# dazzmo/ik

Hardware: AMD Instinct MI355X
Metric: IK solves/sec (50-iter DLS) at batch=65536 (higher is better)
Workload: dtype f64; 1 GPU; Cassie single-leg chain (cassie_fixed.urdf, 7 support joints of nq=16), one SE(3) LeftFootFront task, 50 fixed DLS iterations, damping 1e-2, step 1.0, reachable targets FK(q*); batch_per_gpu=65536, global_batch=65536, kernel=dls_chain<NJ=7,full,hot>, parallelism=single GPU

## Files before the change

### ik_amd/csrc/capi.cpp

```cpp
#include <hip/hip_runtime.h>

#include <time.h>

#include <algorithm>
#include <cmath>
#include <cstdio>
#include <cstdlib>
#include <cstring>
#include <exception>
#include <memory>
#include <mutex>
#include <new>
#include <stdexcept>
#include <string>
#include <type_traits>
#include <vector>

#include "ikgpu.h"
#include "kernels.hpp"
#include "model.hpp"
#include "problem.hpp"

namespace {

// ... 64 lines not shown

struct ikgpu_problem {
    mutable Staging stage;
    mutable HostPipe pipe;
    ikgpu::ProblemHost host;
    ikgpu::ProblemHost gen;
    ikgpu::DeviceTables dev;
    int device = 0;
    int nframes = 0;
    bool dls_on_static_gen = false;
    mutable std::once_flag visitor_static_once;
    mutable uint64_t visitor_static_key = 0;
    mutable bool visitor_static = false;
    mutable std::once_flag pik_static_once[2];
    mutable uint64_t pik_static_key[2] = {0, 0};
    mutable bool pik_static[2] = {false, false};
    std::vector<uint8_t> draw;
    std::string dls_name;
    std::string pik_name;
    std::string pik_tree_name;
    std::string pik_static_name;
    explicit ikgpu_problem(int device_) : device(device_) {}
    ~ikgpu_problem() {
        DeviceGuard g(device);
        void *const tables[] = {dev.lower, dev.upper, dev.q_in_chain, dev.draw, dev.chain_desc, dev.g_ints, dev.g_dbls};
        for (void *t : tables) (void)hipFree(t);
        dev.queues.release();
        pipe.release();
        stage.release();
    }
};
static_assert(!std::is_copy_constructible<Staging>::value && !std::is_copy_constructible<HostPipe>::value &&
                  !std::is_copy_constructible<ikgpu_problem>::value && !std::is_copy_assignable<ikgpu_problem>::value,
              "owners of device memory must not be copyable");

namespace {

thread_local std::string g_last_error;

bool shape_built(const ikgpu::ProblemHost &ph) {
    if (ph.kind == ikgpu::KernelKind::Generic) return true;
    return ph.kind == ikgpu::KernelKind::Chain ? ikgpu::chain_shape_built(ph.chain.nj, ph.tasks[0].type)
                                               : ikgpu::tree_shape_built(ph.chain.nj, ph.chainB.nj > 0 ? 2 : 1);
}

ikgpu::ProblemHost analyse(const ikgpu::Model &m, const ikgpu_task *tasks, int32_t ntasks, const ikgpu_task *cons, int32_t ncons,
                           bool compile_rtc) {
    const char *force = std::getenv("IKGPU_DLS_KERNEL");
    ikgpu::ProblemHost ph = ikgpu::analyse_problem(m, tasks, ntasks, force && std::strcmp(force, "generic") == 0, cons, ncons);
    if (!shape_built(ph)) ph = ikgpu::analyse_problem(m, tasks, ntasks, true, cons, ncons);
    if (ph.kind == ikgpu::KernelKind::Chain) {
        ph.chain_build = ikgpu::select_chain_build(ph, compile_rtc);
        ph.kernel_name = ikgpu::chain_kernel_name(ph);
    }
    if (ph.kind == ikgpu::KernelKind::Generic && ikgpu::rtc_generic_static_available(ph, compile_rtc, &ph.generic_key)) {
        ph.generic_build = 2;
        ph.kernel_name = ph.kernel_name.substr(0, ph.kernel_name.size() - 1) + ",static>";
    }
    return ph;
}

int fail(int code, const std::string &msg) {
    g_last_error = msg;
    return code;
}

bool tree_prefers_static(const ikgpu::ProblemHost &ph) {
    if (ph.kind != ikgpu::KernelKind::Tree) return false;
    long rows = 12;
    if (const char *env = std::getenv("IKGPU_TREE_STATIC_ROWS")) rows = std::strtol(env, nullptr, 10);
    if (ph.cons_on && !std::getenv("IKGPU_TREE_STATIC_CONSTRAINED")) return false;
    return ikgpu::rtc_static_solve_rows(ph) <= rows;
}

std::string static_name(const ikgpu::ProblemHost &gen) {
    const std::string &n = gen.kernel_name;
    return n.size() > 8 && n.compare(n.size() - 8, 8, ",static>") == 0 ? n : n.substr(0, n.size() - 1) + ",static>";
}

struct KernelPlan {
    ikgpu::ProblemHost host, gen;
    bool dls_on_static_gen = false;
    std::string name;
};
KernelPlan plan_kernels(const ikgpu::Model &m, const ikgpu_task *tasks, int32_t ntasks, const ikgpu_task *cons, int32_t ncons, bool compile) {
    KernelPlan k;
    k.host = analyse(m, tasks, ntasks, cons, ncons, compile);
    k.gen = k.host.kind == ikgpu::KernelKind::Generic ? k.host : ikgpu::analyse_problem(m, tasks, ntasks, true, cons, ncons);
    k.name = k.host.kernel_name;
    if (tree_prefers_static(k.host) && ikgpu::rtc_generic_static_available(k.gen, compile, &k.gen.generic_key)) {
        k.gen.generic_build = 2;
        k.dls_on_static_gen = true;
        k.name = static_name(k.gen);
    }
    return k;
}

}

int ikgpu_set_last_error(int code, const std::string &msg) { return fail(code, msg); }

namespace {

int hip_fail(hipError_t e, const char *what) {
    return fail(IKGPU_ERR_DEVICE, std::string(what) + ": " + hipGetErrorString(e));
}
// ... 1363 lines not shown
```

### ik_amd/csrc/device/chain_hot.hpp

```cpp
#pragma once
#if !defined(__HIPCC_RTC__)
#include <cstdint>
#endif

#include "chain_kernel_body.hpp"

namespace ikdev {

constexpr int kStructBits = 21;
constexpr int kStructPerWord = 3;
enum : unsigned { kEntGeneral = 0, kEntZero = 1, kEntOne = 2, kEntMinusOne = 3 };

template <uint64_t C0, uint64_t C1, uint64_t C2, unsigned PM = 0>
struct ChainStruct {
    static constexpr unsigned kPrismatic = PM;
    static constexpr bool prismatic(int j) { return j >= 0 && ((PM >> j) & 1u) != 0; }
    static constexpr uint64_t word(int w) { return w == 0 ? C0 : (w == 1 ? C1 : C2); }
    static constexpr unsigned code(int i) { return static_cast<unsigned>((word(i / kStructPerWord) >> (kStructBits * (i % kStructPerWord))) & 0x1fffffu); }
    static constexpr unsigned ent(int i, int e) { return (code(i) >> (2 * e)) & 3u; }
    static constexpr bool tnz(int i, int k) { return ((code(i) >> (18 + k)) & 1u) != 0; }
    static constexpr int ngen_before(int i, int e) { return e == 0 ? 0 : ngen_before(i, e - 1) + (ent(i, e - 1) == kEntGeneral ? 1 : 0); }
    static constexpr int count(int i) { return ngen_before(i, 9) + (tnz(i, 0) ? 1 : 0) + (tnz(i, 1) ? 1 : 0) + (tnz(i, 2) ? 1 : 0); }
    static constexpr int offset(int i) { return i == 0 ? 0 : offset(i - 1) + count(i - 1); }
    static constexpr int rot_at(int i, int e) { return offset(i) + ngen_before(i, e); }
// ... 37 lines not shown
};

struct HotLutNoStage {};
#if IKD_HIP_LANG
typedef double SinCosPair __attribute__((ext_vector_type(2)));
static __device__ const double kSinCosLutDevice[2 * IKD_SINCOS_LUT_SIZE] __attribute__((aligned(16), unused)) = {IKD_SINCOS_LUT_VALUES};
struct HotTableLds : HotTable {
    SinCosPair *lut;
};
constexpr int kHotLutPerLane = IKD_SINCOS_LUT_SIZE / 64;
struct HotLutStage { SinCosPair v[kHotLutPerLane]; };
__device__ __forceinline__ HotLutStage hot_lut_issue(const HotTableLds &) {
    HotLutStage st;
    const SinCosPair *src = reinterpret_cast<const SinCosPair *>(kSinCosLutDevice);
    const int lane = static_cast<int>(threadIdx.x) & 63;
#pragma unroll
    for (int i = 0; i < kHotLutPerLane; ++i) st.v[i] = src[lane + 64 * i];
    return st;
}
__device__ __forceinline__ void hot_lut_commit(const HotTableLds &t, const HotLutStage &st) {
    const int lane = static_cast<int>(threadIdx.x) & 63;
#pragma unroll
    for (int i = 0; i < kHotLutPerLane; ++i) t.lut[lane + 64 * i] = st.v[i];
    __builtin_amdgcn_fence(__ATOMIC_RELEASE, "workgroup");
    __builtin_amdgcn_wave_barrier();
    __builtin_amdgcn_fence(__ATOMIC_ACQUIRE, "workgroup");
}
__device__ __forceinline__ void hot_lut_fetch(const HotTableLds &t, int idx, double &S, double &C) {
    const SinCosPair e = t.lut[idx];
    S = e.x;
    C = e.y;
}
#define IKD_HOT_LUT_DECLARE(tv)                                       \
    __shared__ SinCosPair ikd_hot_lut[IKD_SINCOS_LUT_SIZE];           \
    HotTableLds tv;                                                   \
    tv.lut = ikd_hot_lut
#endif
IKD_FN HotLutNoStage hot_lut_issue(const HotTable &) { return HotLutNoStage{}; }
IKD_FN void hot_lut_commit(const HotTable &, const HotLutNoStage &) {}
#if IKD_ON_DEVICE && !defined(IKD_HOT_LUT_FROM_HBM)
void hot_lut_fetch(const HotTable &, int idx, double &S, double &C) = delete;
#else
IKD_FN void hot_lut_fetch(const HotTable &, int idx, double &S, double &C) {
#if IKD_ON_DEVICE
    S = kSinCosLutDevice[2 * idx];
    C = kSinCosLutDevice[2 * idx + 1];
#else
    S = kSinCosLutHost[2 * idx];
    C = kSinCosLutHost[2 * idx + 1];
#endif
}
#endif

template <int NJ, unsigned PM = 0, class Tab>
IKD_FN void hot_sincos(const Tab &t, const double (&phi)[NJ], double (&sn)[NJ], double (&cs)[NJ]) {
    double res[NJ], tS[NJ], tC[NJ], sl[NJ], cm1[NJ];
    int idx[NJ];
#pragma unroll
    for (int j = 0; j < NJ; ++j)
        if (!((PM >> j) & 1u)) dsincos_lut_reduce(phi[j], res[j], idx[j]);
#pragma unroll
    for (int j = NJ - 1; j >= 0; --j)
        if (!((PM >> j) & 1u)) hot_lut_fetch(t, idx[j], tS[j], tC[j]);
    IKD_SCHED_FENCE();
#pragma unroll
    for (int j = 0; j < NJ; ++j)
        if (!((PM >> j) & 1u)) dsincos_lut_poly(res[j], sl[j], cm1[j]);
#pragma unroll
    for (int j = NJ - 1; j >= 0; --j)
        if (!((PM >> j) & 1u)) dsincos_lut_combine(tS[j], tC[j], sl[j], cm1[j], sn[j], cs[j]);
}

template <class S, int I, class Tab>
IKD_FN double hot_rot(const Tab &t, int e) {
    return S::ent(I, e) == kEntGeneral ? t.v[S::rot_at(I, e)] : S::literal(I, e);
}

template <class S, int I, class Tab>
IKD_FN void hot_compose_left(double (&R)[9], double (&p)[3], const Tab &t) {
    double Ro[9], po[3];
#pragma unroll
    for (int k = 0; k < 9; ++k) Ro[k] = R[k];
#pragma unroll
    for (int k = 0; k < 3; ++k) po[k] = p[k];
#pragma unroll
    for (int r = 0; r < 3; ++r) {
        const double c0 = hot_rot<S, I>(t, 3 * r), c1 = hot_rot<S, I>(t, 3 * r + 1), c2 = hot_rot<S, I>(t, 3 * r + 2);
#pragma unroll
        for (int k = 0; k < 3; ++k) R[3 * r + k] = dfma(c0, Ro[k], dfma(c1, Ro[3 + k], c2 * Ro[6 + k]));
        const double last = S::tnz(I, r) ? dfma(c2, po[2], t.v[S::trans_at(I, r)]) : c2 * po[2];
        p[r] = dfma(c0, po[0], dfma(c1, po[1], last));
    }
}

template <class S, class Tab>
IKD_FN void hot_fold_base(const Tab &t, const double (&oMt)[12], double (&oM0)[12]) {
    double c[9], dp[3];
#pragma unroll
    for (int k = 0; k < 9; ++k) c[k] = hot_rot<S, 0>(t, k);
#pragma unroll
    for (int k = 0; k < 3; ++k) dp[k] = S::tnz(0, k) ? oMt[9 + k] - t.v[S::trans_at(0, k)] : oMt[9 + k];
#pragma unroll
    for (int i = 0; i < 3; ++i) {
#pragma unroll
        for (int j = 0; j < 3; ++j) oM0[3 * i + j] = dfma(c[i], oMt[j], dfma(c[3 + i], oMt[3 + j], c[6 + i] * oMt[6 + j]));
        oM0[9 + i] = dfma(c[i], dp[0], dfma(c[3 + i], dp[1], c[6 + i] * dp[2]));
    }
}

template <int NJ, class S, bool BASE_FOLDED = false, class Tab>
IKD_FN void hot_evaluate(const Tab &t, const double (&q)[NJ], const double (&oMt)[12], double (&e)[6], double (&col)[NJ][6]) {
    constexpr typename ChainRuns<S, NJ>::Table kRuns = ChainRuns<S, NJ>::value;
    double phi[NJ], sn[NJ], cs[NJ];
#pragma unroll
    for (int j = NJ - 1; j >= 0; --j) phi[j] = (kRuns.folded[j] && !kRuns.tip[j]) ? phi[j + 1 < NJ ? j + 1 : j] + q[j] : q[j];
    hot_sincos<NJ, S::kPrismatic>(t, phi, sn, cs);

    double ang[NJ][3], lin[NJ][3];
    double rows[NJ][6], pt[NJ][2];
    double R[9], p[3];
// ... 150 lines not shown
IKD_FN void hot_step(const Tab &t, const LoopParams &prm, const double (&col)[NJ][6], const double (&y)[6], double (&q)[NJ], bool take) {
    constexpr int kLim = S::offset(NJ + 1);
    constexpr typename ChainRuns<S, NJ>::Table kRuns = ChainRuns<S, NJ>::value;
    double ang[NJ];
#pragma unroll
    for (int j = 0; j < NJ; ++j)
        if (kRuns.leader[j] == j && !kRuns.prismatic[j]) ang[j] = dfma(col[j][3], y[3], dfma(col[j][4], y[4], col[j][5] * y[5]));
#pragma unroll
    for (int j = 0; j < NJ; ++j) {
        double s = kRuns.prismatic[j] ? 0.0 : ang[kRuns.leader[j]];
#pragma unroll
        for (int a = 0; a < 3; ++a) s = dfma(col[j][a], y[a], s);
        const double qn = dfma(prm.step_length, s, q[j]);
        const double qc = dmin(t.v[kLim + NJ + j], dmax(qn, t.v[kLim + j]));
        q[j] = take ? qc : q[j];
    }
}

template <int NJ, class S, bool NEVERSTOP, class Tab, class AnyFn>
IKD_FN void hot_dls(const Tab &t, const LoopParams &prm, double (&q)[NJ], const double (&oMt)[12], int &iters_out,
                    bool &success_out, AnyFn any_active, bool active = true) {
    constexpr int M = 6;
    bool success = false;
    int iters = prm.max_iterations;
    double oM0[12];
    hot_fold_base<S>(t, oMt, oM0);
#pragma unroll 1
    for (int it = 0; it < prm.max_iterations; ++it) {
        double e[M], col[NJ][M];
        hot_evaluate<NJ, S, true>(t, q, oM0, e, col);

        double G[M * M];
        hot_gram<NJ, S>(col, prm.lam2, G);
        double y[M];
        ldlt_solve<M>(G, e, y);

        if (!NEVERSTOP) {
            double e0sq = 0.0;
            if (prm.priority == 0) {
#pragma unroll
                for (int a = 0; a < M; ++a) e0sq = dfma(e[a], e[a], e0sq);
            }
            const bool stop_now = active && (prm.stop_sq_tol >= 0.0) && (e0sq < prm.stop_sq_tol);
            if (stop_now) { success = true; iters = it; }
            active = active && !stop_now;
        }
        hot_step<NJ, S>(t, prm, col, y, q, NEVERSTOP || active);
        if (!NEVERSTOP && !any_active(active)) break;
    }
    iters_out = (NEVERSTOP || success) ? iters : iterations_taken(any_active, prm.max_iterations);
    success_out = success;
}

template <int NJ>
IKD_FN void hot_pass_through_from(const ChainKernelArgs<NJ> &a, const double *q_src, double *q_out, int64_t b, bool stepped) {
    const ChainStrides st = chain_strides(a);
    constexpr int kGroup = 16;
    for (int i0 = 0; i0 < a.nq; i0 += kGroup) {
        double v[kGroup], lo[kGroup], hi[kGroup];
        bool out[kGroup];
#pragma unroll
        for (int k = 0; k < kGroup; ++k) {
            const int i = i0 + k < a.nq ? i0 + k : a.nq - 1;
            out[k] = i0 + k < a.nq && !a.q_in_chain[i];
            lo[k] = a.lower[i];
            hi[k] = a.upper[i];
        }
#pragma unroll
        for (int k = 0; k < kGroup; ++k) {
            const int i = i0 + k < a.nq ? i0 + k : a.nq - 1;
            v[k] = q_src[at(st.elem, st.q_prob, i, b)];
        }
#pragma unroll
        for (int k = 0; k < kGroup; ++k) {
            const double c = dmin(hi[k], dmax(v[k], lo[k]));
            if (out[k]) q_out[at(st.elem, st.q_prob, i0 + k, b)] = stepped ? c : v[k];
        }
    }
}
template <int NJ>
IKD_FN void hot_pass_through_to(const ChainKernelArgs<NJ> &a, double *q_out, int64_t b, bool stepped) { hot_pass_through_from(a, a.q0, q_out, b, stepped); }
template <int NJ>
IKD_FN void hot_pass_through(const ChainKernelArgs<NJ> &a, int64_t b, bool stepped) { hot_pass_through_to(a, a.q_out, b, stepped); }

#if IKD_HIP_LANG
template <int NJ, class S, class Tab>
__device__ __forceinline__ void hot_refill_body(const ChainKernelArgs<NJ> &a, const Tab &t, unsigned long long *queue, int chunk) {
    struct Stage {
        const Tab &t;
        decltype(hot_lut_issue(t)) st;
        __device__ __forceinline__ void issue() { st = hot_lut_issue(t); }
        __device__ __forceinline__ void commit() { hot_lut_commit(t, st); }
    };
    chain_refill_loop<NJ>(a, queue, chunk, [&](double (&q)[NJ], const double (&oMt)[12], bool have) {
        constexpr int M = 6;
        double e[M], col[NJ][M];
        hot_evaluate<NJ, S, true>(t, q, oMt, e, col);
        double G[M * M];
        hot_gram<NJ, S>(col, a.prm.lam2, G);
        double y[M];
        ldlt_solve<M>(G, e, y);
        double e0sq = 0.0;
        if (a.prm.priority == 0) {
#pragma unroll
            for (int k = 0; k < M; ++k) e0sq = dfma(e[k], e[k], e0sq);
        }
        const bool stop_now = have && (a.prm.stop_sq_tol >= 0.0) && (e0sq < a.prm.stop_sq_tol);
        hot_step<NJ, S>(t, a.prm, col, y, q, !stop_now);
        return stop_now;
    }, [&](double (&oMt)[12]) {
        double w[12];
#pragma unroll
        for (int k = 0; k < 12; ++k) w[k] = oMt[k];
        hot_fold_base<S>(t, w, oMt);
    }, Stage{t, {}});
}
#endif

template <int NJ, class S, bool NEVERSTOP, class Tab, class AnyFn>
IKD_FN void hot_chain_body(const ChainKernelArgs<NJ> &a, const Tab &t, int64_t gid, AnyFn any_active, long long wave_start = 0) {
    const ChainStrides st = chain_strides(a);
#if defined(IKGPU_HOT_STAMP) && IKD_ON_DEVICE
    const long long rs = wave_start;
#endif
    const bool valid = gid < a.B;
    const int64_t b = valid ? gid : a.B - 1;
    const auto lut_stage = hot_lut_issue(t);
    double q[NJ];
#pragma unroll
    for (int j = 0; j < NJ; ++j) q[j] = a.q0[at(st.elem, st.q_prob, a.qidx[j], b)];
    double oMt[12];
    load_target(a, b, oMt);
    hot_lut_commit(t, lut_stage);
    if (NEVERSTOP && valid) hot_pass_through(a, b, a.prm.max_iterations > 0);
    int iters;
    bool success;
#if defined(IKGPU_HOT_STAMP) && IKD_ON_DEVICE
    const long long c0 = __builtin_readcyclecounter(), r0 = wall_clock64();
#endif
    hot_dls<NJ, S, NEVERSTOP>(t, a.prm, q, oMt, iters, success, any_active);
#if defined(IKGPU_HOT_STAMP) && IKD_ON_DEVICE
    const long long c1 = __builtin_readcyclecounter(), r1 = wall_clock64();
    const int stamp_loop_cycles = static_cast<int>(c1 - c0), stamp_loop_ticks = static_cast<int>(r1 - r0);
    const int stamp_pre_ticks = static_cast<int>(r0 - rs);
    const int stamp_true_iters = iters;
#endif
    if (!NEVERSTOP && a.append_count)
        append_unfinished(a.append_list, a.append_count, valid && !success && iters < a.prm.max_iterations, b);
    if (!valid) return;
#pragma unroll
    for (int j = 0; j < NJ; ++j) a.q_out[at(st.elem, st.q_prob, a.qidx[j], b)] = q[j];
    if (!NEVERSTOP) hot_pass_through(a, b, iters > 0);
    if (a.success) a.success[b] = success ? 1 : 0;
#if defined(IKGPU_HOT_STAMP) && IKD_ON_DEVICE
    {
        asm volatile("s_waitcnt vmcnt(0)" ::: "memory");
        const long long re = wall_clock64();
        const int lane = threadIdx.x % 64;
        iters = lane == 0 ? stamp_loop_cycles : lane == 1 ? stamp_loop_ticks : lane == 2 ? stamp_pre_ticks
              : lane == 3 ? static_cast<int>(re - r1) : lane == 4 ? static_cast<int>(rs & 0x7fffffff)
              : lane == 5 ? static_cast<int>(re & 0x7fffffff) : stamp_true_iters;
    }
#endif
    if (a.iters) a.iters[b] = iters;
}

template <int NJ, class S, bool NEVERSTOP, class Tab, class AnyFn>
IKD_FN void hot_track_body(const ChainKernelArgs<NJ> &a, const Tab &t, int T, int64_t gid, AnyFn any_active) {
    const ChainStrides st = chain_strides(a);
    const bool valid = gid < a.B;
    const int64_t b = valid ? gid : a.B - 1;
    const int64_t q_slab = static_cast<int64_t>(a.nq) * a.B, t_slab = 12 * a.B;
    const auto lut_stage = hot_lut_issue(t);
    double q[NJ];
#pragma unroll
    for (int j = 0; j < NJ; ++j) q[j] = a.q0[at(st.elem, st.q_prob, a.qidx[j], b)];
    double next[12], oMt[12];
    if (T > 0) {
        load_target_raw(a, a.targets, b, next);
        compose_target(a, next, oMt);
    }
    if (T > 1) load_target_raw(a, a.targets + t_slab, b, next);
    hot_lut_commit(t, lut_stage);
    bool stepped = NEVERSTOP && a.prm.max_iterations > 0;
    for (int k = 0; k < T; ++k) {
        double *q_out = a.q_out + k * q_slab;
        if (NEVERSTOP && valid) hot_pass_through_to(a, q_out, b, stepped);
// ... 387 lines not shown
```

### ik_amd/csrc/device/chain_kernel_body.hpp

```cpp
#pragma once
#if !defined(__HIPCC_RTC__)
#include <cstdint>
#endif

#include "chain_solver.hpp"
#include "goalset.hpp"
#include "line.hpp"
#include "multistart.hpp"
#include "pick.hpp"
#include "solutions.hpp"

namespace ikdev {

enum : int { LAYOUT_SOA = 0, LAYOUT_AOS = 1 };

template <int NJ>
struct ChainKernelArgs {
    const ChainDesc<NJ> *desc;
    LoopParams prm;
    double ref_pl[12];
    int qidx[NJ];
    int vidx[NJ];
    int nq, nv, layout;
    int64_t B;
    const double *q0;
    const double *targets;
    double *q_out;
    uint8_t *success;
    int32_t *iters;
    const double *lower, *upper;
    const uint8_t *q_in_chain;
    double *e_out, *J_out, *oMf_out;
    const int32_t *worklist;
    const unsigned long long *count;
    int leave_active, leave_after;
    int32_t *append_list;
    unsigned long long *append_count;
};

IKD_FN void append_unfinished(int32_t *list, unsigned long long *count, bool open, int64_t b) {
#if IKD_ON_DEVICE
    const unsigned long long mask = __ballot(open);
    if (mask == 0ull) return;
    const int lane = static_cast<int>(threadIdx.x) & 63;
    unsigned long long base = 0;
    if (lane == __ffsll(static_cast<long long>(mask)) - 1) base = atomicAdd(count, static_cast<unsigned long long>(__popcll(mask)));
    const int src = __ffsll(static_cast<long long>(mask)) - 1;
    const unsigned lo = __shfl(static_cast<unsigned>(base), src), hi = __shfl(static_cast<unsigned>(base >> 32), src);
    base = (static_cast<unsigned long long>(hi) << 32) | lo;
    if (open) list[base + __popcll(mask & ((1ull << lane) - 1ull))] = static_cast<int32_t>(b);
#else
    if (open) list[(*count)++] = static_cast<int32_t>(b);
#endif
}

IKD_FN int64_t at(int layout, int64_t B, int ncomp, int c, int64_t b) {
    return layout == LAYOUT_SOA ? static_cast<int64_t>(c) * B + b : b * ncomp + c;
}

struct ChainStrides {
    int64_t elem, q_prob, t_prob;
};
#if IKD_ON_DEVICE
#define IKD_OPAQUE_S(x) asm("" : "+s"(x))
#else
#define IKD_OPAQUE_S(x) ((void)0)
#endif
template <class Args>
IKD_FN ChainStrides chain_strides(const Args &a) {
    const bool soa = a.layout == LAYOUT_SOA;
    ChainStrides s{soa ? a.B : int64_t{1}, soa ? int64_t{1} : static_cast<int64_t>(a.nq), soa ? int64_t{1} : int64_t{12}};
    IKD_OPAQUE_S(s.elem);
    IKD_OPAQUE_S(s.q_prob);
    IKD_OPAQUE_S(s.t_prob);
    return s;
}
IKD_FN int64_t at(int64_t elem, int64_t prob, int c, int64_t b) { return static_cast<int64_t>(c) * elem + b * prob; }

template <int NJ>
IKD_FN void load_target(const ChainKernelArgs<NJ> &a, int64_t b, double (&oMt)[12]) {
    const ChainStrides st = chain_strides(a);
    double t[12];
#pragma unroll
    for (int k = 0; k < 12; ++k) t[k] = a.targets[at(st.elem, st.t_prob, k, b)];
    const double *r = a.ref_pl;
#pragma unroll
    for (int i = 0; i < 3; ++i) {
#pragma unroll
        for (int j = 0; j < 3; ++j)
            oMt[3 * i + j] = dfma(r[3 * i], t[j], dfma(r[3 * i + 1], t[3 + j], r[3 * i + 2] * t[6 + j]));
// ... 694 lines not shown
```

### ik_amd/csrc/kernels.hpp

```cpp
#pragma once
#include <hip/hip_runtime.h>

#include <cstdint>
#include <mutex>
#include <string>
#include <unordered_map>
#include <vector>

#include "device/goalset.hpp"
#include "device/line.hpp"
#include "device/multistart.hpp"
#include "device/pick.hpp"
#include "device/solutions.hpp"
#include "problem.hpp"

namespace ikgpu {

struct QueuePool {
    static constexpr int kChunkSlots = 256;
    std::mutex mu;
    std::vector<unsigned long long *> chunks;
    int used_in_last = kChunkSlots;
    std::unordered_map<hipStream_t, unsigned long long *> by_stream;
    hipError_t grow();
// ... 153 lines not shown
    if (mode == kStopLockStep) return lockstep();
    const bool two = mode == kStopTwoPhase;
    hipError_t e = hipSuccess;
    unsigned long long *queue = queues.slot_for(stream, &e);
    if (!queue) return e;
    int32_t *list = nullptr;
    if (two) {
        if (io.B > 0x7fffffff) return hipErrorInvalidValue;
        if (!(list = queues.worklist_for(stream, static_cast<size_t>(io.B), &e))) return e;
    }
    void *tmp[2] = {nullptr, nullptr};
    if (two && !a.success && (e = hipMallocAsync(&tmp[0], static_cast<size_t>(io.B), stream)) == hipSuccess)
        a.success = static_cast<uint8_t *>(tmp[0]);
    if (e == hipSuccess && (two || pass_through.ph) && !a.iters &&
        (e = hipMallocAsync(&tmp[1], sizeof(int32_t) * static_cast<size_t>(io.B), stream)) == hipSuccess)
        a.iters = static_cast<int32_t *>(tmp[1]);
    const int chunk = refill_chunk(io.B, resident_waves);
    if (e == hipSuccess && two) {
        unsigned long long *count = queue + 2;
        a.worklist = nullptr; a.count = nullptr;
        a.leave_active = two_phase_active(tree); a.leave_after = two_phase_iterations(tree);
        a.append_list = list; a.append_count = count;
        e = lockstep();
        if (e == hipSuccess) {
            a.leave_active = 0; a.leave_after = 0;
            a.append_list = nullptr; a.append_count = nullptr;
            a.worklist = list; a.count = count;
            e = refill(queue, chunk);
            if (e != hipSuccess) (void)hipMemsetAsync(count, 0, sizeof(*count), stream);
        }
    } else if (e == hipSuccess) {
        e = refill(queue, chunk);
        if (e == hipSuccess && pass_through.ph) e = launch_chain_pass_through(*pass_through.ph, *pass_through.dt, io, a.iters, stream);
    }
    for (void *p : tmp)
        if (p) { const hipError_t f = hipFreeAsync(p, stream); if (e == hipSuccess) e = f; }
    return e;
}

template <class A>
inline void fill_solve_args(A &a, const BatchIO &io, const ikgpu_dls_params &prm) {
    a.prm.max_iterations = prm.max_iterations;
    a.prm.lam2 = prm.damping * prm.damping;
    a.prm.step_length = prm.step_length;
    a.prm.stop_sq_tol = prm.stop_sq_tol;
    a.layout = io.layout; a.B = io.B; a.q0 = io.q0; a.targets = io.targets;
    a.q_out = io.q_out; a.success = io.success; a.iters = io.iters;
}
template <class A>
inline void fill_chain_kernel_args(A &a, const ProblemHost &ph, const DeviceTables &dt) {
    fill_chain_args(ph, a.ref_pl, a.qidx, a.vidx, &a.nq, &a.nv, &a.prm.priority, &a.prm.idmask, &a.prm.unit_weights);
    a.desc = reinterpret_cast<decltype(a.desc)>(dt.chain_desc);
    a.lower = dt.lower; a.upper = dt.upper; a.q_in_chain = dt.q_in_chain;
}
bool rtc_chain_hot_available(const ProblemHost &ph, bool compile);
bool rtc_generic_static_available(const ProblemHost &gen, bool compile, uint64_t *key_out);
hipError_t rtc_launch_generic_static(const ProblemHost &gen, uint64_t key, const BatchIO &io, const ikgpu_dls_params &prm, hipStream_t stream,
                                     QueuePool &queues);
int rtc_static_solve_rows(const ProblemHost &ph);
bool rtc_generic_static_precompile_refill(const ProblemHost &gen);
bool rtc_pik_static_available(const ProblemHost &gen, bool with_da, bool compile, uint64_t *key_out);
hipError_t rtc_launch_pik_static(const ProblemHost &gen, uint64_t key, const BatchIO &io, const ikgpu_pik_params &prm, hipStream_t stream);
std::string rtc_last_log();
hipError_t rtc_launch_chain_hot(const ProblemHost &ph, const DeviceTables &dt, const BatchIO &io, const ChainJob &job, const ikgpu_dls_params &prm,
                                hipStream_t stream);
hipError_t launch_targets_from_pose7(int64_t B, int ntasks, const double *pose7, double *targets12, int layout, hipStream_t stream);
int64_t persistent_grid(const void *kernel, int block, size_t lds, int64_t nblocks);
bool raise_lds_limit(const void *kernel, size_t lds, size_t limit = 160 * 1024);
hipError_t launch_dls_chain_hot(const ProblemHost &ph, const DeviceTables &dt, const BatchIO &io, const ChainJob &job, const ikgpu_dls_params &prm,
                                hipStream_t stream);

}

namespace ikgpu {
hipError_t launch_dls_tree(const ProblemHost &ph, const DeviceTables &dt, const BatchIO &io,
                           const ikgpu_dls_params &prm, hipStream_t stream, const double *pik_lambda1 = nullptr);
bool tree_takes_two_level_pik(const ProblemHost &ph);
hipError_t launch_eval_tree(const ProblemHost &ph, const DeviceTables &dt, int64_t B, const double *q,
                            const double *targets, double *e_out, double *J_out, double *oMf_out, int layout,
                            hipStream_t stream);
bool tree_shape_built(int nj, int nch);
bool generic_runs_cooperative(const ProblemHost &ph);
hipError_t launch_dls_generic(const ProblemHost &ph, const DeviceTables &dt, const BatchIO &io,
                              const ikgpu_dls_params &prm, hipStream_t stream, bool force_lane = false);
hipError_t launch_pik_generic(const ProblemHost &gen, const DeviceTables &dt, const BatchIO &io, const ikgpu_pik_params &prm,
                              hipStream_t stream);
hipError_t launch_eval_generic(const ProblemHost &ph, const DeviceTables &dt, int64_t B, const double *q,
                               const double *targets, double *e_out, double *J_out, double *oMf_out, int layout,
                               hipStream_t stream);
}
```

### ik_amd/csrc/kernels_hot.hip

```cpp
#include "kernels.hpp"

#include <cstdlib>
#include <cstring>
#include <type_traits>

#include "device/chain_hot.hpp"

namespace ikgpu {
namespace {

constexpr int kBlock = 64;

using ikdev::ChainKernelArgs;
using ikdev::ChainStruct;
using ikdev::HotTable;

template <int NJ, uint64_t C0, uint64_t C1, uint64_t C2, bool NEVERSTOP>
__global__ __launch_bounds__(kBlock) void dls_chain_hot_kernel(const ChainKernelArgs<NJ> a, const HotTable t) {
    ikdev::hot_kernel_entry<NJ, ChainStruct<C0, C1, C2>, NEVERSTOP>(a, t);
}

#ifndef IKGPU_HOT_REFILL_WAVES
#define IKGPU_HOT_REFILL_WAVES 2
#endif
template <int NJ, uint64_t C0, uint64_t C1, uint64_t C2>
__global__ __launch_bounds__(kBlock, IKGPU_HOT_REFILL_WAVES) void dls_chain_hot_refill_kernel(const ChainKernelArgs<NJ> a, const HotTable t, unsigned long long *queue, int chunk) {
    ikdev::hot_refill_entry<NJ, ChainStruct<C0, C1, C2>>(a, t, queue, chunk);
}

template <int NJ, uint64_t C0, uint64_t C1, uint64_t C2, bool NEVERSTOP>
__global__ __launch_bounds__(kBlock) void dls_chain_hot_track_kernel(const ChainKernelArgs<NJ> a, const HotTable t, const int T) {
    ikdev::hot_track_entry<NJ, ChainStruct<C0, C1, C2>, NEVERSTOP>(a, t, T);
}

template <int NJ, uint64_t C0, uint64_t C1, uint64_t C2, bool NEVERSTOP>
__global__ __launch_bounds__(kBlock) void dls_chain_hot_multistart_kernel(const ChainKernelArgs<NJ> a, const HotTable t, const ikdev::MultistartArgs ms) {
    ikdev::hot_multistart_entry<NJ, ChainStruct<C0, C1, C2>, NEVERSTOP>(a, t, ms);
}

template <int NJ, uint64_t C0, uint64_t C1, uint64_t C2>
__global__ __launch_bounds__(kBlock) void dls_chain_hot_pick_kernel(const ChainKernelArgs<NJ> a, const HotTable t, const ikdev::PickArgs pk) {
    ikdev::hot_pick_entry<NJ, ChainStruct<C0, C1, C2>>(a, t, pk);
}

template <int NJ, uint64_t C0, uint64_t C1, uint64_t C2>
__global__ __launch_bounds__(kBlock) void dls_chain_hot_path_multistart_kernel(const ChainKernelArgs<NJ> a, const HotTable t,
                                                                               const ikdev::PathMultistartArgs pm) {
    ikdev::hot_path_multistart_entry<NJ, ChainStruct<C0, C1, C2>>(a, t, pm);
}

template <int NJ, uint64_t C0, uint64_t C1, uint64_t C2, bool NEVERSTOP>
__global__ __launch_bounds__(kBlock) void dls_chain_hot_goalset_kernel(const ChainKernelArgs<NJ> a, const HotTable t, const ikdev::GoalsetArgs ga) {
    ikdev::hot_goalset_entry<NJ, ChainStruct<C0, C1, C2>, NEVERSTOP>(a, t, ga);
}

template <int NJ, uint64_t C0, uint64_t C1, uint64_t C2>
__global__ __launch_bounds__(kBlock) void dls_chain_hot_solutions_kernel(const ChainKernelArgs<NJ> a, const HotTable t, const ikdev::SolutionsArgs sa) {
    ikdev::hot_solutions_entry<NJ, ChainStruct<C0, C1, C2>>(a, t, sa);
}

template <int NJ, uint64_t C0, uint64_t C1, uint64_t C2>
__global__ __launch_bounds__(kBlock) void dls_chain_hot_line_kernel(const ChainKernelArgs<NJ> a, const HotTable t, const ikdev::LineArgs la) {
    ikdev::hot_line_entry<NJ, ChainStruct<C0, C1, C2>>(a, t, la);
}

template <int NJ, uint64_t C0, uint64_t C1, uint64_t C2>
__global__ __launch_bounds__(kBlock) void dls_chain_hot_path_kernel(const ChainKernelArgs<NJ> a, const HotTable t, const ikdev::PathArgs pa) {
    ikdev::hot_path_entry<NJ, ChainStruct<C0, C1, C2>>(a, t, pa);
// ... 107 lines not shown
```

### ik_amd/csrc/problem.cpp

```cpp
#include "problem.hpp"

#include <algorithm>
#include <cmath>
#include <cstdlib>
#include <cstring>
#include <stdexcept>
#include <type_traits>

#include "device/tree_kernel_body.hpp"

namespace ikgpu {
namespace {

void axis_frame(const std::array<double, 3> &a, double *P) {
    auto set = [&](std::initializer_list<double> v) { int i = 0; for (double x : v) P[i++] = x; };
    if (a == std::array<double, 3>{0, 0, 1}) { set({1, 0, 0, 0, 1, 0, 0, 0, 1}); return; }
    if (a == std::array<double, 3>{1, 0, 0}) { set({0, 0, 1, 0, 1, 0, -1, 0, 0}); return; }
    if (a == std::array<double, 3>{0, 1, 0}) { set({1, 0, 0, 0, 0, 1, 0, -1, 0}); return; }
    int k = 0;
    if (std::fabs(a[1]) < std::fabs(a[k])) k = 1;
    if (std::fabs(a[2]) < std::fabs(a[k])) k = 2;
    double t[3] = {0, 0, 0};
    t[k] = 1.0;
    double b1[3] = {t[1] * a[2] - t[2] * a[1], t[2] * a[0] - t[0] * a[2], t[0] * a[1] - t[1] * a[0]};
// ... 48 lines not shown
    return c;
}

void weights6(const ikgpu_task &t, double *w6) {
    for (int i = 0; i < 6; ++i) w6[i] = 0.0;
    if (t.type == IKGPU_FULL) for (int i = 0; i < 6; ++i) w6[i] = t.weight[i];
    if (t.type == IKGPU_POSITION) for (int i = 0; i < 3; ++i) w6[i] = t.weight[i];
    if (t.type == IKGPU_ORIENTATION) for (int i = 0; i < 3; ++i) w6[3 + i] = t.weight[i];
}

}

namespace {

struct Unsupported : std::runtime_error {
    using std::runtime_error::runtime_error;
};

void specialise(ProblemHost &ph, const Model &m) {
    static const char *kt[] = {"position", "orientation", "full"};
    const int ntasks = ph.ntasks;
    const bool free_flyer = m.njoints() > 1 && m.joint_type[1] == IKGPU_JOINT_FREEFLYER;
    for (const ikgpu_task &t : ph.tasks) {
        if (t.type == IKGPU_CENTRE_OF_MASS) throw Unsupported("CentreOfMassTask rows run on the generic kernel");
    }
    for (int j = 1; j < m.njoints(); ++j)
        if (m.joint_type[j] == IKGPU_JOINT_REVOLUTE_UNBOUNDED) throw Unsupported("a model with continuous joints runs on the generic kernel");
    std::vector<uint8_t> in_chain(m.nq, 0);

    auto chain_of = [&](const std::vector<int> &joints, int frame, int task_index, bool prismatic_ok = false) {
        if (static_cast<int>(joints.size()) > kMaxChain) throw Unsupported("support chain longer than the specialised kernels take");
        for (int j : joints) {
            if (m.joint_type[j] != IKGPU_JOINT_REVOLUTE && !(prismatic_ok && m.joint_type[j] == IKGPU_JOINT_PRISMATIC))
                throw Unsupported("non-revolute joint in a task support");
            if (in_chain[m.joint_idx_q[j]]) throw Unsupported("a joint is in the support of two tasks");
        }
        return build_chain(m, joints, frame, task_index, in_chain, prismatic_ok);
    };

    if (!ph.constraints.empty() && !free_flyer) throw Unsupported("a constraint on a fixed-base model runs on the generic kernel");
    if (!free_flyer && ntasks == 1 && ph.tasks[0].type <= IKGPU_FULL) {
        const ikgpu_task &t = ph.tasks[0];
        if (m.frame_parent[t.reference] != 0) throw Unsupported("reference frame moves with the configuration");
        std::memcpy(ph.ref_pl, m.frame_placement[t.reference].data(), sizeof(double) * 12);
        std::vector<int> joints;
        for (int j = m.frame_parent[t.frame]; j > 0; j = m.joint_parent[j]) joints.insert(joints.begin(), j);
        if (joints.empty()) throw Unsupported("task frame fixed in the world");
        ph.chain = chain_of(joints, t.frame, 0, true);
        ph.chain_struct = chain_structure(ph.chain);
        ph.chain_hot = chain_hot_table(ph.chain);
        ph.kind = KernelKind::Chain;
        ph.kernel_name = "dls_chain<NJ=" + std::to_string(ph.chain.nj) + "," + kt[t.type] + ",general>";
        ph.q_in_chain = in_chain;
        return;
    }
    const int root = free_flyer ? 1 : 0;
    ph.fixed_base = !free_flyer;
    if (free_flyer)
        for (int k = 0; k < 7; ++k) in_chain[k] = 1;
    int nchains = 0;
    int chain_frame[2] = {-1, -1};
    for (int i = 0; i < ntasks; ++i) {
        const ikgpu_task &t = ph.tasks[i];
        if (t.type > IKGPU_FULL) continue;
        const bool ref_world = m.frame_parent[t.reference] == 0 && is_identity(m.frame_placement[t.reference]);
        const bool ref_on_base = free_flyer && m.frame_parent[t.reference] == 1;
        if (!ref_world && !ref_on_base) throw Unsupported("reference frame neither the universe nor on the floating base");
        if (m.frame_parent[t.frame] == 0) throw Unsupported("task frame fixed in the world");
        std::vector<int> joints;
        for (int j = m.frame_parent[t.frame]; j > root; j = m.joint_parent[j]) joints.insert(joints.begin(), j);
        if (joints.empty()) {
            if (ph.base_task >= 0) throw Unsupported("two tasks on the floating base link");
            if (!ref_world) throw Unsupported("base-link task with a reference frame other than the universe");
            ph.base_task = i;
            std::memcpy(ph.base_frame_pl, m.frame_placement[t.frame].data(), sizeof(double) * 12);
        } else {
            if (nchains == 2) throw Unsupported("more than two chain tasks on a free-flyer model");
            (nchains == 0 ? ph.chain : ph.chainB) = chain_of(joints, t.frame, i);
            if (ref_on_base) {
                ph.ref_base[nchains] = 1;
                std::memcpy(ph.chain_ref_pl[nchains], m.frame_placement[t.reference].data(), sizeof(double) * 12);
            }
            chain_frame[nchains] = t.frame;
            ++nchains;
        }
    }
    for (int i = 0; i < ntasks; ++i) {
        const ikgpu_task &t = ph.tasks[i];
        if (t.type <= IKGPU_FULL || t.type == IKGPU_POSTURE_ROW) continue;
        if (ph.align_task >= 0) throw Unsupported("more than one AlignAxisTask");
        if (m.frame_parent[t.reference] != 0 || !is_identity(m.frame_placement[t.reference]))
            throw Unsupported("AlignAxisTask with a reference frame other than the universe");
        const int c = t.frame == chain_frame[0] ? 0 : (t.frame == chain_frame[1] ? 1 : -1);
        if (c < 0) throw Unsupported("AlignAxisTask on a frame that carries no frame task");
        ph.align_task = i;
        ph.align_chain = c;
    }
    if (nchains == 0) throw Unsupported("free-flyer problem without a chain task");
    if (!ph.constraints.empty()) {
        const ikgpu_task &c = ph.constraints[0];
        if (ph.constraints.size() != 1) throw Unsupported("more than one constraint");
        if (nchains != 1) throw Unsupported("a constraint next to two chain tasks");
        if (m.frame_parent[c.reference] != 0 || !is_identity(m.frame_placement[c.reference]))
            throw Unsupported("constraint with a reference frame other than the universe");
        std::vector<int> joints;
        for (int j = m.frame_parent[c.frame]; j > root; j = m.joint_parent[j]) joints.insert(joints.begin(), j);
// ... 259 lines not shown
    for (int j = 0; j < nj; ++j) put_d(m.joint_axis[j].data(), 3);
    g.o_lower = put_d(m.lower.data(), m.lower.size());
    g.o_upper = put_d(m.upper.data(), m.upper.size());
    g.o_tfpl = static_cast<int>(g.dbls.size());
    const SE3 ident = se3_identity();
    for (int i = 0; i < nt; ++i)
        put_d(ph.tasks[i].type == IKGPU_POSTURE_ROW || ph.tasks[i].type == IKGPU_CENTRE_OF_MASS ? ident.data()
                                                                                              : m.frame_placement[ph.tasks[i].frame].data(), 12);
    g.o_trpl = static_cast<int>(g.dbls.size());
    for (int i = 0; i < nt; ++i)
        put_d(ph.tasks[i].type == IKGPU_POSTURE_ROW ? ident.data() : m.frame_placement[ph.tasks[i].reference].data(), 12);
    g.o_tw = static_cast<int>(g.dbls.size());
    for (int i = 0; i < nt; ++i) put_d(ph.tasks[i].weight, 6);
    {
        std::vector<double> sub(m.joint_mass);
        if (!sub.empty()) sub[0] = 0.0;
        for (int j = nj - 1; j > 0; --j) sub[m.joint_parent[j]] += sub[j];
        g.o_jmass = put_d(m.joint_mass.data(), m.joint_mass.size());
        g.o_jlever = static_cast<int>(g.dbls.size());
        for (int j = 0; j < nj; ++j) put_d(m.joint_com[j].data(), 3);
        g.o_jsubmass = put_d(sub.data(), sub.size());
        g.inv_total_mass = sub.empty() || !(sub[0] > 0.0) ? 0.0 : 1.0 / sub[0];
    }
    g.o_cfpl = static_cast<int>(g.dbls.size());
    for (const ikgpu_task &c : ph.constraints) put_d(m.frame_placement[c.frame].data(), 12);
    g.o_crpl = static_cast<int>(g.dbls.size());
    for (const ikgpu_task &c : ph.constraints) put_d(m.frame_placement[c.reference].data(), 12);
    const int M = ph.rows, nv = m.nv;
    int o = 0;
    g.off_q = o; o += m.nq;
    g.off_oMi = o; o += 12 * nj;
    g.off_Jw = o; o += 6 * nv;
    g.off_e = o; o += M;
    g.off_J = o; o += M * nv;
    g.off_G = o; o += M * (M + 1) / 2;
    g.off_y = o; o += M;
    g.off_dq = o; o += nv;
    g.off_Jc = o; o += crows * nv;
    g.off_sf = o; o += g.has_com ? 3 * nj : 0;
    g.ws_words = o;
    build_coop(ph, m);
    g.off_P = o; o += nv * nv;
    g.off_Jb = o; o += mmax * nv;
    g.off_de = o; o += mmax;
    g.ws_words_pik = o;
    ph.kind = KernelKind::Generic;
    ph.kernel_name = "dls_generic<M=" + std::to_string(M) + ",nv=" + std::to_string(nv) + ",joints=" + std::to_string(nj - 1) +
                     (crows > 0 ? ",constraint_rows=" + std::to_string(crows) : std::string()) + ">";
    ph.q_in_chain.assign(m.nq, 1);
}

}

ProblemHost analyse_problem(const Model &m, const ikgpu_task *tasks, int ntasks, bool force_generic,
                            const ikgpu_task *constraints, int nconstraints) {
    if (ntasks < 1) throw std::runtime_error("a problem needs at least one task");
    if (nconstraints < 0 || (nconstraints > 0 && !constraints)) throw std::runtime_error("invalid constraint list");
    ProblemHost ph;
    for (int i = 0; i < nconstraints; ++i) {
        const ikgpu_task &c = constraints[i];
        if (c.frame < 0 || c.frame >= m.nframes()) throw std::runtime_error("constraint " + std::to_string(i) + ": frame id out of range");
        if (c.reference < 0 || c.reference >= m.nframes())
            throw std::runtime_error("constraint " + std::to_string(i) + ": reference frame id out of range");
        if (c.type < IKGPU_POSITION || c.type > IKGPU_FULL)
            throw std::runtime_error("constraint " + std::to_string(i) + ": a frame constraint is of type Position, Orientation or Full");
        ph.constraints.push_back(c);
        ph.crows += task_dim(c);
    }
    if (nconstraints > 1) force_generic = true;
    ph.nq = m.nq;
    ph.nv = m.nv;
    ph.ntasks = ntasks;
    ph.lower = m.lower;
    ph.upper = m.upper;
    ph.q_in_chain.assign(m.nq, 0);
    int last_prio = 0;
    for (int i = 0; i < ntasks; ++i) {
        const ikgpu_task &t = tasks[i];
        if (t.type == IKGPU_CENTRE_OF_MASS) {
            if (t.reference < 0 || t.reference >= m.nframes()) throw std::runtime_error("task " + std::to_string(i) + ": reference frame id out of range");
            if (!(m.total_mass() > 0.0))
                throw std::runtime_error("task " + std::to_string(i) + ": a centre-of-mass task needs joint masses (the model has none)");
        } else if (t.type == IKGPU_POSTURE_ROW) {
            if (t.frame < 0 || t.frame >= m.nv) throw std::runtime_error("task " + std::to_string(i) + ": posture row tangent index out of range");
            if (t.reference < 0 || t.reference >= m.nq) throw std::runtime_error("task " + std::to_string(i) + ": posture row configuration index out of range");
        } else {
            if (t.frame < 0 || t.frame >= m.nframes()) throw std::runtime_error("task " + std::to_string(i) + ": frame id out of range");
            if (t.reference < 0 || t.reference >= m.nframes()) throw std::runtime_error("task " + std::to_string(i) + ": reference frame id out of range");
        }
        if (t.type < IKGPU_POSITION || t.type > IKGPU_CENTRE_OF_MASS) throw std::runtime_error("task " + std::to_string(i) + ": unknown kinematic type");
        if (t.priority < 0) throw std::runtime_error("task " + std::to_string(i) + ": negative priority");
        if (t.priority < last_prio) throw std::runtime_error("tasks must be listed in stacking order (non-decreasing priority)");
        last_prio = t.priority;
        ph.tasks.push_back(t);
        ph.task_row.push_back(ph.rows);
        ph.rows += task_dim(t);
    }
    if (!force_generic) {
        try {
            ProblemHost sp = ph;
            specialise(sp, m);
            return sp;
        } catch (const Unsupported &) {
        }
    }
    build_generic(ph, m);
// ... 235 lines not shown
```

### ik_amd/csrc/problem.hpp

```cpp
#pragma once
#include <cstdint>
#include <string>
#include <vector>

#include "ikgpu.h"
#include "model.hpp"

namespace ikgpu {

constexpr int kMaxChain = 8;
constexpr int kMaxPostureOut = 32;

enum class KernelKind { Chain, Tree, Generic };

struct GenericHost {
    std::vector<int32_t> ints;
    std::vector<double> dbls;
    int o_jtype = 0, o_parent = 0, o_idx_q = 0, o_idx_v = 0;
    int o_ttype = 0, o_tfjoint = 0, o_trjoint = 0, o_trow = 0, o_tdim = 0, o_tprio = 0;
    int o_placement = 0, o_axis = 0, o_lower = 0, o_upper = 0, o_tfpl = 0, o_trpl = 0, o_tw = 0;
    int njoints = 0;
    int off_q = 0, off_oMi = 0, off_Jw = 0, off_e = 0, off_J = 0, off_G = 0, off_y = 0, off_dq = 0, ws_words = 0;
    int nlevels = 1, o_lvlrow0 = 0;
    int off_P = 0, off_Jb = 0, off_de = 0, ws_words_pik = 0;
    int o_ctype = 0, o_cfjoint = 0, o_crjoint = 0, o_crow = 0, o_cdim = 0;
    int o_ccpair_i = 0, o_ccpair_j = 0;
    int o_cfpl = 0, o_crpl = 0;
    int off_Jc = 0;
    int coop_ok = 0, coop_rounds = 0, coop_words = 0, coop_npairs = 0, coop_nblocks = 0, o_cbtask = 0;
    int coop_post_elim = 0, coop_Mf = 0, c_Dd = 0, o_cfrow = 0, o_cpstart = 0, o_cptask = 0;
    int d_words = 0, d_A1 = 0, d_Jw = 0, d_e = 0, d_dq = 0, d_Dd = 0, d_sf = 0, d_J = 0, d_G = 0, o_cjrow = 0;
    int coop_ntg = 0, o_ctgoff = 0, o_ctgsrc = 0;
    int coop_pik_ok = 0, coop_words_pik = 0, coop_mmax = 0, c_P = 0;
    int o_csupport = 0, o_cpair_i = 0, o_cpair_j = 0, o_cup = 0, o_cchain = 0, o_clvl = 0, o_ctbindex = 0, o_ccoljoint = 0, o_ccsf = 0, o_ccsr = 0;
    int c_q = 0, c_tg = 0, c_A0 = 0, c_A1 = 0, c_Jw = 0, c_tb = 0, c_e = 0, c_J = 0, c_G = 0, c_dinv = 0, c_x = 0, c_dq = 0, c_sf = 0, c_cb = 0, c_Jc = 0, c_cnrm = 0;
    int has_com = 0, o_jmass = 0, o_jlever = 0, o_jsubmass = 0, off_sf = 0;
    double inv_total_mass = 0.0;
};

struct ChainHost {
    int nj = 0;
    int prismatic = 0;
    int task = -1;
    int qidx[kMaxChain] = {};
    int vidx[kMaxChain] = {};
    double pl[kMaxChain][12] = {};
    double frame_pl[12] = {};
    double lo[kMaxChain] = {}, hi[kMaxChain] = {};
};

struct ChainStructure {
    uint64_t code[3] = {0, 0, 0};
    bool fits = false;
    int values = 0;
    int prismatic = 0;
};
ChainStructure chain_structure(const ChainHost &c);
std::vector<double> chain_hot_table(const ChainHost &c);

struct ProblemHost {
    KernelKind kind = KernelKind::Chain;
    std::string kernel_name;
    int nq = 0, nv = 0, ntasks = 0, rows = 0;
    std::vector<ikgpu_task> tasks;
    std::vector<int> task_row;
    ChainHost chain;
    ChainStructure chain_struct;
    std::vector<double> chain_hot;
    int chain_build = 0;
    int generic_build = 0;
    uint64_t generic_key = 0;
    ChainHost chainB;
    int base_task = -1;
    double base_frame_pl[12] = {};
    double ref_pl[12] = {};
    int ref_base[2] = {0, 0};
    double chain_ref_pl[2][12] = {{1, 0, 0, 0, 1, 0, 0, 0, 1, 0, 0, 0}, {1, 0, 0, 0, 1, 0, 0, 0, 1, 0, 0, 0}};
    int align_task = -1, align_chain = -1;
    struct PostureRow { int task, qi; double w, mask; };
    bool has_posture = false;
    int posture_prio = 0;
    std::vector<PostureRow> posture_out;
    int posture_chain_task[2][kMaxChain];
    double posture_chain_w[2][kMaxChain] = {}, posture_chain_mask[2][kMaxChain] = {};
    bool fixed_base = false;
    bool cons_on = false;
    int cons_type = 0;
    bool tree_extras() const { return ref_base[0] || ref_base[1] || align_task >= 0 || has_posture || fixed_base || cons_on; }
    GenericHost generic;
    std::vector<ikgpu_task> constraints;
    int crows = 0;
    std::vector<uint8_t> q_in_chain;
    std::vector<double> lower, upper;
};

ProblemHost analyse_problem(const Model &m, const ikgpu_task *tasks, int ntasks, bool force_generic = false,
                            const ikgpu_task *constraints = nullptr, int nconstraints = 0);

std::vector<double> chain_desc_table(const ProblemHost &ph);
std::vector<double> tree_desc_table(const ProblemHost &ph);
void fill_chain_args(const ProblemHost &ph, double *ref_pl12, int *qidx, int *vidx, int *nq, int *nv, int *priority,
                     int *idmask, int *unit_weights);
int chain_identity_mask(const ChainHost &c);
int chain_kernel_mask(const ChainHost &c);
bool task_has_unit_weights(const ikgpu_task &t);
struct TreeArgsHost {
    int qidx[2][kMaxChain], vidx[2][kMaxChain];
    int tslot[3], trow[3], tdim[3], trow0[3];
    int prio[3];
    int hasP, nch;
    int idmask[2], idmaskP, unit[3];
    int ref_base[2];
    int align_chain, align_axis, align_slot, align_prio;
    double align_w;
    int fixed_base;
    int cons_on, cons_type;
    int post_on, post_prio, post_n;
    int post_q[kMaxPostureOut], post_slot[kMaxPostureOut];
    double post_w[kMaxPostureOut], post_m[kMaxPostureOut];
    int postc_slot[2][kMaxChain];
    double postc_w[2][kMaxChain], postc_m[2][kMaxChain];
};
TreeArgsHost tree_args(const ProblemHost &ph);

struct TreeBuild {
    enum { kHot = 0, kHotNever, kMask, kGeneral };
    enum { kNone = 0, kPosture, kConstraint, kPostureConstraint, kPik };
    enum { kRefillNone = 0, kRefillHot, kRefillMask, kRefillFold, kRefillGeneral };
    int build = kGeneral;
    bool folded = false;
    int extras = kNone;
    int refill = kRefillNone;
    bool launchable = true;
};
TreeBuild select_tree_build(const ProblemHost &ph, const ikgpu_dls_params &prm, bool pik);
std::string tree_build_name(const TreeBuild &b);

std::vector<uint8_t> multistart_draw_mask(const Model &m, const ProblemHost &ph);

}
```

Before: 769.6 million solves/s.

## Precompute pass-through joint plan on host and prefetch pass-through q early

Builds a host-side plan listing the joints outside the chain together with their limits, and passes it in kernel arguments. The hot kernel then issues the pass-through q loads at kernel start and commits the clamped writes later. This replaces the generic loop over all nq joints, which read q_in_chain, lower and upper from global memory. It also adds an explicit lgkmcnt(0) wait before the sincos combine, and it enlarges the kernarg struct.

```diff
diff --git a/ik_amd/csrc/capi.cpp b/ik_amd/csrc/capi.cpp
--- a/ik_amd/csrc/capi.cpp
+++ b/ik_amd/csrc/capi.cpp
@@ -140,6 +140,8 @@
     if (ph.kind == ikgpu::KernelKind::Chain) {
         ph.chain_build = ikgpu::select_chain_build(ph, compile_rtc);
         ph.kernel_name = ikgpu::chain_kernel_name(ph);
+        const char *plan = std::getenv("IKGPU_HOT_PASS_PLAN");
+        if (plan && std::strcmp(plan, "0") == 0) ph.pass_plan = ikgpu::PassPlanHost{};
     }
     if (ph.kind == ikgpu::KernelKind::Generic && ikgpu::rtc_generic_static_available(ph, compile_rtc, &ph.generic_key)) {
         ph.generic_build = 2;
diff --git a/ik_amd/csrc/device/chain_hot.hpp b/ik_amd/csrc/device/chain_hot.hpp
--- a/ik_amd/csrc/device/chain_hot.hpp
+++ b/ik_amd/csrc/device/chain_hot.hpp
@@ -113,6 +113,16 @@
 }
 #endif
 
+constexpr int kWaitLgkm0 = 0xc07f;
+#if IKD_ON_DEVICE
+#define IKD_LDS_LANDED()                                                                   \
+    do {                                                                                   \
+        __builtin_amdgcn_s_waitcnt(kWaitLgkm0);                                            \
+        IKD_SCHED_FENCE();                                                                 \
+    } while (0)
+#else
+#define IKD_LDS_LANDED() ((void)0)
+#endif
 template <int NJ, unsigned PM = 0, class Tab>
 IKD_FN void hot_sincos(const Tab &t, const double (&phi)[NJ], double (&sn)[NJ], double (&cs)[NJ]) {
     double res[NJ], tS[NJ], tC[NJ], sl[NJ], cm1[NJ];
@@ -127,6 +137,7 @@
 #pragma unroll
     for (int j = 0; j < NJ; ++j)
         if (!((PM >> j) & 1u)) dsincos_lut_poly(res[j], sl[j], cm1[j]);
+    IKD_LDS_LANDED();
 #pragma unroll
     for (int j = NJ - 1; j >= 0; --j)
         if (!((PM >> j) & 1u)) dsincos_lut_combine(tS[j], tC[j], sl[j], cm1[j], sn[j], cs[j]);
@@ -383,8 +394,54 @@
     success_out = success;
 }
 
+struct PassStage {
+    double v[kPassPlanMax];
+};
+#if IKD_ON_DEVICE
+#define IKD_PASS_PLAN(name, a, NJ)                                                                                                     \
+    const IKD_CONST_AS char *name##_at = (const IKD_CONST_AS char *)__builtin_amdgcn_kernarg_segment_ptr() +                             \
+                                         __builtin_offsetof(ChainKernelArgs<NJ>, pass);                                                  \
+    IKD_LAUNDER(name##_at);                                                                                                            \
+    const IKD_CONST_AS PassPlan &name = *reinterpret_cast<const IKD_CONST_AS PassPlan *>(name##_at)
+#else
+#define IKD_PASS_PLAN(name, a, NJ) const PassPlan &name = (a).pass
+#endif
+template <int NJ>
+IKD_FN void hot_pass_issue(const ChainKernelArgs<NJ> &a, const double *q_src, int64_t b, PassStage &s) {
+    const ChainStrides st = chain_strides(a);
+#pragma unroll
+    for (int g = 0; g < kPassPlanMax; g += kPassPlanGroup) {
+        if (g < a.pass.n) {
+            IKD_PASS_PLAN(plan, a, NJ);
+#pragma unroll
+            for (int k = g; k < g + kPassPlanGroup; ++k) s.v[k] = q_src[at(st.elem, st.q_prob, plan.idx[k], b)];
+        }
+    }
+}
+template <int NJ>
+IKD_FN void hot_pass_commit(const ChainKernelArgs<NJ> &a, const PassStage &s, double *q_out, int64_t b, bool stepped) {
+    const ChainStrides st = chain_strides(a);
+#pragma unroll
+    for (int g = 0; g < kPassPlanMax; g += kPassPlanGroup) {
+        if (g < a.pass.n) {
+            IKD_PASS_PLAN(plan, a, NJ);
+#pragma unroll
+            for (int k = g; k < g + kPassPlanGroup; ++k) {
+                const double c = dmin(plan.hi[k], dmax(s.v[k], plan.lo[k]));
+                q_out[at(st.elem, st.q_prob, plan.idx[k], b)] = stepped ? c : s.v[k];
+            }
+        }
+    }
+}
+
 template <int NJ>
 IKD_FN void hot_pass_through_from(const ChainKernelArgs<NJ> &a, const double *q_src, double *q_out, int64_t b, bool stepped) {
+    if (a.pass.have) {
+        PassStage s;
+        hot_pass_issue(a, q_src, b, s);
+        hot_pass_commit(a, s, q_out, b, stepped);
+        return;
+    }
     const ChainStrides st = chain_strides(a);
     constexpr int kGroup = 16;
     for (int i0 = 0; i0 < a.nq; i0 += kGroup) {
@@ -456,6 +513,9 @@
 #endif
     const bool valid = gid < a.B;
     const int64_t b = valid ? gid : a.B - 1;
+    const bool planned = NEVERSTOP && a.pass.have;
+    PassStage pass_stage;
+    if (planned) hot_pass_issue(a, a.q0, b, pass_stage);
     const auto lut_stage = hot_lut_issue(t);
     double q[NJ];
 #pragma unroll
@@ -463,7 +523,10 @@
     double oMt[12];
     load_target(a, b, oMt);
     hot_lut_commit(t, lut_stage);
-    if (NEVERSTOP && valid) hot_pass_through(a, b, a.prm.max_iterations > 0);
+    if (NEVERSTOP && valid) {
+        if (planned) hot_pass_commit(a, pass_stage, a.q_out, b, a.prm.max_iterations > 0);
+        else hot_pass_through(a, b, a.prm.max_iterations > 0);
+    }
     int iters;
     bool success;
 #if defined(IKGPU_HOT_STAMP) && IKD_ON_DEVICE
diff --git a/ik_amd/csrc/device/chain_kernel_body.hpp b/ik_amd/csrc/device/chain_kernel_body.hpp
--- a/ik_amd/csrc/device/chain_kernel_body.hpp
+++ b/ik_amd/csrc/device/chain_kernel_body.hpp
@@ -13,6 +13,14 @@
 namespace ikdev {
 
 enum : int { LAYOUT_SOA = 0, LAYOUT_AOS = 1 };
+
+constexpr int kPassPlanMax = 16;
+constexpr int kPassPlanGroup = 8;
+struct PassPlan {
+    int have, n;
+    int idx[kPassPlanMax];
+    double lo[kPassPlanMax], hi[kPassPlanMax];
+};
 
 template <int NJ>
 struct ChainKernelArgs {
@@ -36,6 +44,7 @@
     int leave_active, leave_after;
     int32_t *append_list;
     unsigned long long *append_count;
+    PassPlan pass;
 };
 
 IKD_FN void append_unfinished(int32_t *list, unsigned long long *count, bool open, int64_t b) {
diff --git a/ik_amd/csrc/kernels.hpp b/ik_amd/csrc/kernels.hpp
--- a/ik_amd/csrc/kernels.hpp
+++ b/ik_amd/csrc/kernels.hpp
@@ -229,6 +229,9 @@
     fill_chain_args(ph, a.ref_pl, a.qidx, a.vidx, &a.nq, &a.nv, &a.prm.priority, &a.prm.idmask, &a.prm.unit_weights);
     a.desc = reinterpret_cast<decltype(a.desc)>(dt.chain_desc);
     a.lower = dt.lower; a.upper = dt.upper; a.q_in_chain = dt.q_in_chain;
+    static_assert(sizeof a.pass.idx == sizeof ph.pass_plan.idx && sizeof a.pass.lo == sizeof ph.pass_plan.lo, "PassPlan / PassPlanHost capacity");
+    a.pass.have = ph.pass_plan.have; a.pass.n = ph.pass_plan.n;
+    for (int k = 0; k < kPassPlanMax; ++k) { a.pass.idx[k] = ph.pass_plan.idx[k]; a.pass.lo[k] = ph.pass_plan.lo[k]; a.pass.hi[k] = ph.pass_plan.hi[k]; }
 }
 bool rtc_chain_hot_available(const ProblemHost &ph, bool compile);
 bool rtc_generic_static_available(const ProblemHost &gen, bool compile, uint64_t *key_out);
diff --git a/ik_amd/csrc/kernels_hot.hip b/ik_amd/csrc/kernels_hot.hip
--- a/ik_amd/csrc/kernels_hot.hip
+++ b/ik_amd/csrc/kernels_hot.hip
@@ -14,6 +14,7 @@
 using ikdev::ChainKernelArgs;
 using ikdev::ChainStruct;
 using ikdev::HotTable;
+static_assert(ikdev::kPassPlanMax == kPassPlanMax && ikdev::kPassPlanGroup == kPassPlanGroup, "problem.hpp PassPlanHost is padded for the device's groups");
 
 template <int NJ, uint64_t C0, uint64_t C1, uint64_t C2, bool NEVERSTOP>
 __global__ __launch_bounds__(kBlock) void dls_chain_hot_kernel(const ChainKernelArgs<NJ> a, const HotTable t) {
diff --git a/ik_amd/csrc/problem.cpp b/ik_amd/csrc/problem.cpp
--- a/ik_amd/csrc/problem.cpp
+++ b/ik_amd/csrc/problem.cpp
@@ -124,6 +124,7 @@
         ph.kind = KernelKind::Chain;
         ph.kernel_name = "dls_chain<NJ=" + std::to_string(ph.chain.nj) + "," + kt[t.type] + ",general>";
         ph.q_in_chain = in_chain;
+        ph.pass_plan = pass_through_plan(ph.q_in_chain, ph.lower, ph.upper);
         return;
     }
     const int root = free_flyer ? 1 : 0;
@@ -489,6 +490,27 @@
 
 }
 
+PassPlanHost pass_through_plan(const std::vector<uint8_t> &q_in_chain, const std::vector<double> &lower, const std::vector<double> &upper) {
+    PassPlanHost p;
+    size_t outside = 0;
+    for (uint8_t in : q_in_chain) outside += in ? 0 : 1;
+    if (outside > static_cast<size_t>(kPassPlanMax)) return p;
+    p.have = 1;
+    for (size_t i = 0; i < q_in_chain.size(); ++i) {
+        if (q_in_chain[i]) continue;
+        p.idx[p.n] = static_cast<int>(i);
+        p.lo[p.n] = lower[i];
+        p.hi[p.n] = upper[i];
+        ++p.n;
+    }
+    for (; p.n % kPassPlanGroup != 0; ++p.n) {
+        p.idx[p.n] = p.idx[p.n - 1];
+        p.lo[p.n] = p.lo[p.n - 1];
+        p.hi[p.n] = p.hi[p.n - 1];
+    }
+    return p;
+}
+
 ProblemHost analyse_problem(const Model &m, const ikgpu_task *tasks, int ntasks, bool force_generic,
                             const ikgpu_task *constraints, int nconstraints) {
     if (ntasks < 1) throw std::runtime_error("a problem needs at least one task");
diff --git a/ik_amd/csrc/problem.hpp b/ik_amd/csrc/problem.hpp
--- a/ik_amd/csrc/problem.hpp
+++ b/ik_amd/csrc/problem.hpp
@@ -58,6 +58,14 @@
 ChainStructure chain_structure(const ChainHost &c);
 std::vector<double> chain_hot_table(const ChainHost &c);
 
+constexpr int kPassPlanMax = 16, kPassPlanGroup = 8;
+struct PassPlanHost {
+    int have = 0, n = 0;
+    int idx[kPassPlanMax] = {};
+    double lo[kPassPlanMax] = {}, hi[kPassPlanMax] = {};
+};
+PassPlanHost pass_through_plan(const std::vector<uint8_t> &q_in_chain, const std::vector<double> &lower, const std::vector<double> &upper);
+
 struct ProblemHost {
     KernelKind kind = KernelKind::Chain;
     std::string kernel_name;
@@ -92,6 +100,7 @@
     int crows = 0;
     std::vector<uint8_t> q_in_chain;
     std::vector<double> lower, upper;
+    PassPlanHost pass_plan;
 };
 
 ProblemHost analyse_problem(const Model &m, const ikgpu_task *tasks, int ntasks, bool force_generic = false,
```

After: 776.5 million solves/s (median of 6 runs). About the same (+0.9%).
